# jorr3/Alphazero-4-player-chess

Hardware: AMD Instinct MI355X
Metric: MCTS simulations/sec (whole node), 256 games×400 sims, 10-block ResNet (higher is better)
Workload: dtype fp16

## Files before the change

### alphazero-4-player-chess_amd/csrc/fpc_tower.h

```cpp
#pragma once
#include <hip/hip_runtime.h>

#include <type_traits>

#include "fpc_tree_kernels.h"

namespace fpc {

typedef __attribute__((ext_vector_type(8))) __bf16 t_bf16x8;
typedef __attribute__((ext_vector_type(8))) _Float16 t_f16x8;
typedef __attribute__((ext_vector_type(4))) float t_f32x4;
typedef __attribute__((ext_vector_type(2))) float t_f32x2;
typedef __attribute__((ext_vector_type(4))) uint32_t t_u32x4;
typedef __attribute__((ext_vector_type(2))) uint32_t t_u32x2;
typedef __attribute__((ext_vector_type(2))) short t_i16x2;

template <int DT>
struct M16;
template <>
struct M16<0> {
  static __device__ __forceinline__ t_f32x4 mfma(t_u32x4 a, t_u32x4 b, t_f32x4 c) {
    return __builtin_amdgcn_mfma_f32_16x16x32_bf16(__builtin_bit_cast(t_bf16x8, a), __builtin_bit_cast(t_bf16x8, b), c, 0, 0, 0);
  }
  static __device__ __forceinline__ uint32_t pack2(float lo, float hi) {
    typedef __attribute__((ext_vector_type(2))) __bf16 b2;
    return __builtin_bit_cast(uint32_t, __builtin_convertvector((t_f32x2{lo, hi}), b2));
  }
  static __device__ __forceinline__ float lo(uint32_t p) { return __builtin_bit_cast(float, p << 16); }
  static __device__ __forceinline__ float hi(uint32_t p) { return __builtin_bit_cast(float, p & 0xffff0000u); }
};
template <>
struct M16<1> {
  static __device__ __forceinline__ t_f32x4 mfma(t_u32x4 a, t_u32x4 b, t_f32x4 c) {
    return __builtin_amdgcn_mfma_f32_16x16x32_f16(__builtin_bit_cast(t_f16x8, a), __builtin_bit_cast(t_f16x8, b), c, 0, 0, 0);
  }
  static __device__ __forceinline__ uint32_t pack2(float lo, float hi) {
    typedef __attribute__((ext_vector_type(2))) _Float16 h2;
    return __builtin_bit_cast(uint32_t, __builtin_convertvector((t_f32x2{lo, hi}), h2));
  }
  static __device__ __forceinline__ float lo(uint32_t p) { return (float)__builtin_bit_cast(_Float16, (uint16_t)(p & 0xffffu)); }
  static __device__ __forceinline__ float hi(uint32_t p) { return (float)__builtin_bit_cast(_Float16, (uint16_t)(p >> 16)); }
};
__device__ __forceinline__ uint32_t tw_relu2(uint32_t p) {
  return __builtin_bit_cast(uint32_t, __builtin_elementwise_max(__builtin_bit_cast(t_i16x2, p), (t_i16x2{0, 0})));
}

__host__ __device__ constexpr int tw_lay(int CH, int row, int c) {
  return (row >> 3) * (CH * 128) + (c >> 1) * 256 + (c & 1) * 128 + (row & 7) * 16;
}

constexpr int TW_THREADS = 256;
constexpr int TW_BIAS = 0;
constexpr int TW_DUMMY = 2048;
constexpr int TW_VRED = 2560;
constexpr int TW_BOARD = 2624;
constexpr int TW_PACE = 2944;
constexpr int TW_IMG0 = 4096;
constexpr int TW_IMG = 61440;
constexpr int TW_TAP = 32768;
constexpr int TW_RING = TW_IMG0 + TW_IMG;
constexpr int TW_LDS = TW_RING + 3 * TW_TAP;
constexpr int TW_STEM_TAP = 8192;
constexpr int TW_ENC = TW_RING + 9 * TW_STEM_TAP;
static_assert(TW_LDS == 163840, "k_tower uses the whole LDS of a CU");

struct TowerArgs {
  const fpc_board *boards;
  const int *leaf_slot, *leaf_turn;
  int board_stride;
  uint16_t one16;
  const uint16_t *in16;
  const unsigned char *Wstem;
  const float *bstem;
  const unsigned char *Wt;
  const float *bt;
  uint16_t *xfc;
  const float *vw;
  float *value;
  float vb;
  int L, P, R, PP, NR, T0, n_games, Kp, A_ch;
  int rules;
  unsigned long long *stamps;
};

__device__ __forceinline__ void tw_dma_8k(const unsigned char *gsrc_uniform, uint32_t lane_off, uint32_t lds_addr_uniform) {
  uint32_t keep;
  asm volatile(
      "s_mov_b32 %0, m0\n\ts_mov_b32 m0, %3\n\ts_nop 0\n\t"
      "global_load_lds_dwordx4 %1, %2\n\ts_add_u32 m0, m0, 0x400\n\tv_add_u32 %1, 0x400, %1\n\t"
      "global_load_lds_dwordx4 %1, %2\n\ts_add_u32 m0, m0, 0x400\n\tv_add_u32 %1, 0x400, %1\n\t"
      "global_load_lds_dwordx4 %1, %2\n\ts_add_u32 m0, m0, 0x400\n\tv_add_u32 %1, 0x400, %1\n\t"
      "global_load_lds_dwordx4 %1, %2\n\ts_add_u32 m0, m0, 0x400\n\tv_add_u32 %1, 0x400, %1\n\t"
      "global_load_lds_dwordx4 %1, %2\n\ts_add_u32 m0, m0, 0x400\n\tv_add_u32 %1, 0x400, %1\n\t"
      "global_load_lds_dwordx4 %1, %2\n\ts_add_u32 m0, m0, 0x400\n\tv_add_u32 %1, 0x400, %1\n\t"
      "global_load_lds_dwordx4 %1, %2\n\ts_add_u32 m0, m0, 0x400\n\tv_add_u32 %1, 0x400, %1\n\t"
      "global_load_lds_dwordx4 %1, %2\n\t"
      "s_mov_b32 m0, %0"
      : "=&s"(keep), "+v"(lane_off) : "s"(gsrc_uniform), "s"(lds_addr_uniform) : "memory", "scc");
}
__device__ __forceinline__ void tw_dma_4k(const unsigned char *gsrc_uniform, uint32_t lane_off, uint32_t lds_addr_uniform) {
  uint32_t keep;
  asm volatile(
      "s_mov_b32 %0, m0\n\ts_mov_b32 m0, %3\n\ts_nop 0\n\t"
      "global_load_lds_dwordx4 %1, %2\n\ts_add_u32 m0, m0, 0x400\n\tv_add_u32 %1, 0x400, %1\n\t"
      "global_load_lds_dwordx4 %1, %2\n\ts_add_u32 m0, m0, 0x400\n\tv_add_u32 %1, 0x400, %1\n\t"
      "global_load_lds_dwordx4 %1, %2\n\ts_add_u32 m0, m0, 0x400\n\tv_add_u32 %1, 0x400, %1\n\t"
      "global_load_lds_dwordx4 %1, %2\n\t"
      "s_mov_b32 m0, %0"
      : "=&s"(keep), "+v"(lane_off) : "s"(gsrc_uniform), "s"(lds_addr_uniform) : "memory", "scc");
}
template <int OFF>
__device__ __forceinline__ void tw_dma_piece(const unsigned char *gsrc_uniform, uint32_t lane_off) {
  asm volatile("global_load_lds_dwordx4 %0, %1 offset:%2" : : "v"(lane_off), "s"(gsrc_uniform), "i"(OFF) : "memory");
}
__device__ __forceinline__ void tw_set_m0(uint32_t lds_addr_uniform) {
  asm volatile("s_mov_b32 m0, %0\n\ts_nop 0" : : "s"(lds_addr_uniform) : "memory");
}
__device__ __forceinline__ void tw_dma_256(const unsigned char *gsrc_uniform, uint32_t lane_off, uint32_t lds_addr_uniform) {
  uint32_t keep;
  asm volatile("s_mov_b32 %0, m0\n\ts_mov_b32 m0, %3\n\ts_nop 0\n\tglobal_load_lds_dword %1, %2\n\ts_mov_b32 m0, %0"
               : "=&s"(keep) : "v"(lane_off), "s"(gsrc_uniform), "s"(lds_addr_uniform) : "memory");
}

#ifdef TW_STAMPS
#define TW_STAMP(GT, I)                                                                                       \
  do {                                                                                                        \
    if (g.stamps && blockIdx.x == 0 && ((GT) == TW_STAMPS || (GT) == TW_STAMPS + 1)) {                        \
      const unsigned long long t_ = __builtin_amdgcn_s_memtime();                                             \
      if (lane == 0) g.stamps[(((GT) - TW_STAMPS) * 8 + wave) * 16 + (I)] = t_;                               \
    }                                                                                                         \
  } while (0)
#else
#define TW_STAMP(GT, I) do {} while (0)
#endif
#ifndef TW_AHEAD
#define TW_AHEAD 2
#endif
#ifndef TW_LOADERS
#define TW_LOADERS 1
#endif
#ifndef TW_STAGGER
#define TW_STAGGER 3
#endif
#ifndef TW_STRIP
#define TW_STRIP 0
#endif
#ifndef TWC_LOADER_TILES
#define TWC_LOADER_TILES 6
#endif

#ifndef TWC_STAGGER
#define TWC_STAGGER 2
#endif

template <int DT, int MT, bool FAST, int NW, int LOAD, bool CMP = false, bool TU = false>
__device__ __forceinline__ void tw_body(const TowerArgs &g) {
  static_assert(!CMP || (!FAST && NW == 8 && TW_LOADERS == 1 && MT == (LOAD == 2 ? TWC_LOADER_TILES : 13 - TWC_LOADER_TILES)), "compact form: 8 waves, 13 row tiles");
  static_assert(!TU || (CMP && TW_STAGGER != 0 && TWC_STAGGER >= 1 && TWC_STAGGER <= 3), "tap-specialised loop: compact form with the burst stream");
  constexpr int CR = 14, CZ = 16;
  constexpr int TB0 = LOAD == 2 ? 0 : TWC_LOADER_TILES;
  constexpr int NT = NW * 64;
  constexpr int WN = NW / 2;
  constexpr int CT = 8 / WN;
  constexpr int PIECES = 4 * LOAD;
  constexpr int DMA_PER_WAVE = PIECES * 1024;
  constexpr int MID = PIECES == 8 ? 4096 : 0;
  constexpr bool STREAM = TW_AHEAD == 2 && !(TW_STAGGER != 0 && NW == 8 && TW_LOADERS == 1);
  constexpr int STAG = (NW == 8 && TW_LOADERS == 1 && LOAD == 0) ? (TU ? TWC_STAGGER : TW_STAGGER) : 0;
  extern __shared__ __attribute__((aligned(16))) unsigned char smem[];
  unsigned char *const img = smem + TW_IMG0;
  unsigned char *const ring = smem + TW_RING;
  const float *const biasbuf = reinterpret_cast<const float *>(smem + TW_BIAS);
  float *const vred = reinterpret_cast<float *>(smem + TW_VRED);
  fpc_board *const lboard = reinterpret_cast<fpc_board *>(smem + TW_BOARD);
  const int tid = threadIdx.x, lane = tid & 63;
  const int wave = __builtin_amdgcn_readfirstlane(tid >> 6);
  const int wm = wave / WN, wn = wave % WN;
  const int li = lane & 15, lq = lane >> 4;
  const int game = blockIdx.x;
  const int P = g.P, NR = g.NR;

  int slot = 0, rot_k = 0;
  if (g.boards) {
    slot = g.leaf_slot[game];
    if (slot < 0) return;
    rot_k = first_leaf_turn(g.leaf_slot, g.leaf_turn, g.n_games);
  }

  const int rbase = CMP ? CZ + TB0 * 16 + li : (g.T0 + wm * MT) * 16 + li;
  uint32_t inmask = 0;
#pragma unroll
  for (int mt = 0; mt < MT; ++mt) {
    const int r = rbase + 16 * mt;
    if (CMP) {
      if (r - CZ < CR * CR) inmask |= 1u << mt;
    } else {
      const int pi = r / P, pj = r - pi * P;
      if (r < g.PP && pi >= 1 && pi <= g.R && pj >= 1 && pj <= g.R) inmask |= 1u << mt;
    }
  }
  auto colmask = [](int mt, int dx) -> uint64_t {
    uint32_t m16 = 0;
    for (int i = 0; i < 16; ++i)
      if (dx != 0 && ((TB0 + mt) * 16 + i) % CR == (dx < 0 ? 0 : CR - 1)) m16 |= 1u << i;
    const uint32_t m32 = m16 * 0x10001u;
    return ((uint64_t)m32 << 32) | m32;
  };
  auto lane_select = [](uint32_t a, uint32_t b, uint64_t m) -> uint32_t {
    uint32_t r;
    asm("v_cndmask_b32_e64 %0, %1, %2, %3" : "=v"(r) : "v"(a), "v"(b), "s"(m));
    return r;
  };
  const int bq = (lq >> 1) * 256 + (lq & 1) * 128;
  const int apart = (li >> 3) * 2048 + (li & 7) * 16 + bq;
  const int apart_s = (li >> 3) * 512 + (li & 7) * 16 + bq;
  const int cb64 = wn * (CT * 16);
  const int cb16 = (wn & 1) * 16;
  const bool vactive = wn < 2;

  for (int c = tid; c < (TW_IMG0 + TW_IMG) / 16; c += NT) reinterpret_cast<t_u32x4 *>(smem)[c] = t_u32x4{0u, 0u, 0u, 0u};
  unsigned char *const enc = smem + TW_ENC;
  const int enc_bytes = CMP ? 240 * 64 : ((NR + 7) >> 3) * 512;
  for (int c = tid; c < enc_bytes / 16; c += NT) reinterpret_cast<t_u32x4 *>(enc)[c] = t_u32x4{0u, 0u, 0u, 0u};
  {
    const t_u32x4 *src = reinterpret_cast<const t_u32x4 *>(g.Wstem);
    t_u32x4 *dst = reinterpret_cast<t_u32x4 *>(ring);
    for (int c = tid; c < 9 * TW_STEM_TAP / 16; c += NT) dst[c] = src[c];
  }
  t_f32x4 bst[CT];
#pragma unroll
  for (int ct = 0; ct < CT; ++ct) bst[ct] = *reinterpret_cast<const t_f32x4 *>(g.bstem + cb64 + ct * 16 + 4 * lq);
  __syncthreads();
  if (g.boards) {
    constexpr int WPB = (int)(sizeof(fpc_board) / 4);
    if (tid < WPB) reinterpret_cast<uint32_t *>(lboard)[tid] =
        reinterpret_cast<const uint32_t *>(g.boards + (size_t)game * g.board_stride + slot)[tid];
    __syncthreads();
    if (g.rules & FPC_RULES_ROTATION) rot_k = lboard->turn;
    for (int r = tid; r < (CMP ? CR * CR : g.PP); r += NT) {
      const int pi = CMP ? r / CR + 1 : r / P, pj = CMP ? r % CR + 1 : r - pi * P;
      if (pi < 1 || pi > g.R || pj < 1 || pj > g.R) continue;
      const uint8_t p = lboard->sq[rot90_src(g.R, rot_k, pi - 1, pj - 1)];
      if (!present(p)) continue;
      const int plane = piece_plane(p, lboard->turn, g.rules);
      *reinterpret_cast<uint16_t *>(enc + tw_lay(4, CMP ? CZ + r : r, plane >> 3) + (plane & 7) * 2) = g.one16;
    }
  } else if (CMP) {
    const uint16_t *src = g.in16 + (size_t)game * g.PP * 32;
    for (int c = tid; c < CR * CR * 4; c += NT) {
      const int q = c >> 2, j = c & 3;
      *reinterpret_cast<t_u32x4 *>(enc + tw_lay(4, CZ + q, j)) =
          *reinterpret_cast<const t_u32x4 *>(src + ((size_t)(q / CR + 1) * P + q % CR + 1) * 32 + j * 8);
    }
  } else {
    const uint16_t *src = g.in16 + (size_t)game * g.PP * 32;
    for (int c = tid; c < NR * 4; c += NT) {
      const int r = c >> 2, j = c & 3;
      *reinterpret_cast<t_u32x4 *>(enc + tw_lay(4, r, j)) = *reinterpret_cast<const t_u32x4 *>(src + (size_t)r * 32 + j * 8);
    }
  }
  __syncthreads();

  t_f32x4 acc[MT][CT];
  t_u32x2 res[MT][CT];

  auto brow = [&](int mt, int shift) -> int {
    int r = rbase + 16 * mt + shift;
    r = r < 0 ? r + NR : r;
    r = r >= NR ? r - NR : r;
    return r;
  };

#pragma unroll
  for (int tap = 0; tap < 9; ++tap) {
    const int shift = (tap / 3 - 1) * (CMP ? CR : P) + (tap % 3 - 1);
    t_u32x4 fa[CT], fb[MT];
#pragma unroll
    for (int ct = 0; ct < CT; ++ct)
      fa[ct] = *reinterpret_cast<const t_u32x4 *>(ring + tap * TW_STEM_TAP + (cb64 + ct * 16) * 64 + apart_s);
#pragma unroll
    for (int mt = 0; mt < MT; ++mt) {
      const int r = CMP ? (int)lane_select((uint32_t)(rbase + 16 * mt + shift), (uint32_t)((rbase + shift) & 7), colmask(mt, tap % 3 - 1)) : brow(mt, shift);
      fb[mt] = *reinterpret_cast<const t_u32x4 *>(enc + (r >> 3) * 512 + (r & 7) * 16 + bq);
    }
#pragma unroll
    for (int mt = 0; mt < MT; ++mt)
#pragma unroll
      for (int ct = 0; ct < CT; ++ct) acc[mt][ct] = M16<DT>::mfma(fa[ct], fb[mt], tap == 0 ? bst[ct] : acc[mt][ct]);
  }
  __syncthreads();

  const int total = (g.L + 2) * 9;
  const uint32_t dma_lane = (uint32_t)lane * 16u;
  const int lw = LOAD == 2 ? (wave & 3) : wave;
  auto issue_bias = [&](int T) {
    if (T % 9 == 0 && T < total && wave < 4) {
      const int l = T / 9;
      tw_dma_256(reinterpret_cast<const unsigned char *>(g.bt + (size_t)l * 256 + wave * 64), (uint32_t)lane * 4u,
                 (uint32_t)__builtin_amdgcn_readfirstlane(TW_BIAS + ((l & 1) * 256 + wave * 64) * 4));
    }
  };
  auto issue_tap = [&](int T) {
    issue_bias(T);
    if (LOAD == 0 || (TW_STRIP & 4)) return;
    const unsigned char *src = g.Wt + (size_t)T * TW_TAP + lw * DMA_PER_WAVE;
    const uint32_t dst = (uint32_t)__builtin_amdgcn_readfirstlane(TW_RING + (T % 3) * TW_TAP + lw * DMA_PER_WAVE);
    if (PIECES == 8) tw_dma_8k(src, dma_lane, dst);
    else tw_dma_4k(src, dma_lane, dst);
  };
  const unsigned char *dsrc = g.Wt;
  auto open_tap = [&](int T) {
    issue_bias(T);
    if (LOAD == 0) return;
    dsrc = g.Wt + (size_t)T * TW_TAP + lw * DMA_PER_WAVE + MID;
    tw_set_m0((uint32_t)__builtin_amdgcn_readfirstlane(TW_RING + (T % 3) * TW_TAP + lw * DMA_PER_WAVE + MID));
  };
  auto piece = [&](auto i_c) {
    constexpr int I = decltype(i_c)::value;
    if (LOAD != 0) tw_dma_piece<I * 1024 - MID>(dsrc, dma_lane);
  };
  issue_tap(0);
  issue_tap(1);
  if (STREAM) {
    open_tap(2);
    piece(std::integral_constant<int, 0>{});
    if (LOAD == 2) piece(std::integral_constant<int, 1>{});
  }

  unsigned char *const dummy = smem + TW_DUMMY + lane * 8;
  unsigned char *const wbase = img + (rbase >> 3) * 2048 + (rbase & 7) * 16 + wn * (CT * 256) + (lane >> 5) * 128 + ((lane >> 4) & 1) * 8;
  auto epilogue = [&](auto res_c) {
    constexpr int RES = decltype(res_c)::value;
    if (TW_STRIP & 16) return;
#pragma unroll
    for (int mt = 0; mt < MT; ++mt) {
      unsigned char *dst = ((inmask >> mt) & 1u) ? wbase + mt * 4096 : dummy;
#pragma unroll
      for (int ct = 0; ct < CT; ++ct) {
        t_f32x4 v = acc[mt][ct];
        if (RES == 2) {
          v[0] += M16<DT>::lo(res[mt][ct][0]); v[1] += M16<DT>::hi(res[mt][ct][0]);
          v[2] += M16<DT>::lo(res[mt][ct][1]); v[3] += M16<DT>::hi(res[mt][ct][1]);
        }
        const t_u32x2 pk = t_u32x2{tw_relu2(M16<DT>::pack2(v[0], v[1])), tw_relu2(M16<DT>::pack2(v[2], v[3]))};
        if (RES != 0) res[mt][ct] = pk;
        *reinterpret_cast<t_u32x2 *>(((inmask >> mt) & 1u) ? dst + ct * 256 : dst) = pk;
      }
      __builtin_amdgcn_sched_barrier(0);
    }
  };
  const std::integral_constant<int, 0> c0{};
  const std::integral_constant<int, 1> c1{};
  const std::integral_constant<int, 2> c2{};
  const std::integral_constant<int, 3> c3{};
  epilogue(c1);
  if (TW_STRIP & 32) { asm volatile("s_waitcnt vmcnt(0)" ::: "memory"); return; }
  if (STREAM) asm volatile("s_waitcnt vmcnt(%0)" ::"n"(PIECES + LOAD) : "memory");
  else asm volatile("s_waitcnt vmcnt(0)" ::: "memory");
  __syncthreads();

  t_u32x4 fa[2][CT], fb[2][MT];
  int gt = 0;
  const unsigned char *wslot;
  const unsigned char *bbase;
  const unsigned char *blast;
  int boff[FAST ? 1 : MT];
  auto set_tap = [&](int tap, int cb) {
    wslot = ring + (gt % 3) * TW_TAP + cb * 256 + apart;
    const int shift = (tap / 3 - 1) * P + (tap % 3 - 1);
    if (FAST) {
      const int r = rbase + shift;
      bbase = img + (r >> 3) * 2048 + (r & 7) * 16 + bq;
      int rl = r + 16 * (MT - 1);
      rl = rl >= NR ? rl - NR : rl;
      blast = img + (rl >> 3) * 2048 + (rl & 7) * 16 + bq;
    } else if (CMP) {
      const int dx = tap % 3 - 1;
      const int r = rbase + (tap / 3 - 1) * CR + dx;
      const uint32_t zoff = (r & 7) * 16 + bq;
      const uint32_t b0 = (r >> 3) * 2048 + zoff;
#pragma unroll
      for (int mt = 0; mt < MT; ++mt) {
        const uint64_t m = dx < 0 ? colmask(mt, -1) : dx > 0 ? colmask(mt, 1) : 0ull;
        boff[mt] = (int)lane_select(b0 + mt * 4096, zoff, m);
      }
    } else {
#pragma unroll
      for (int mt = 0; mt < MT; ++mt) {
        const int r = brow(mt, shift);
        boff[mt] = (r >> 3) * 2048 + (r & 7) * 16 + bq;
      }
    }
  };
  const unsigned char *wrow = nullptr, *wrow2 = nullptr;
  auto set_wrow = [&](int cb) {
    int o = cb * 256 + apart, o2 = o + 2 * TW_TAP;
    asm volatile("" : "+v"(o2));
    wrow = ring + o;
    wrow2 = ring + o2;
  };
  int rrow = rbase - CR;
  auto set_tap_u = [&](auto xn_c) {
    constexpr int XN = decltype(xn_c)::value;
    wslot = XN == 2 ? wrow2 : wrow + XN * TW_TAP;
    const int r = rrow + (XN - 1);
    const uint32_t zoff = (r & 7) * 16 + bq;
    const uint32_t b0 = (r >> 3) * 2048 + zoff;
#pragma unroll
    for (int mt = 0; mt < MT; ++mt)
      boff[mt] = XN == 1 ? (int)(b0 + mt * 4096) : (int)lane_select(b0 + mt * 4096, zoff, colmask(mt, XN - 1));
  };
  auto bptr = [&](int mt) -> const unsigned char * {
    if (FAST) return mt == MT - 1 ? blast : bbase + mt * 4096;
    return img + boff[mt];
  };
  auto kstep = [&](auto mode_c, auto buf_c, auto ksn_c, auto bias_c, const t_f32x4 *b4, auto q_c) {
    constexpr int MODE = decltype(mode_c)::value, B = decltype(buf_c)::value, KSN = decltype(ksn_c)::value;
    constexpr bool BIAS = decltype(bias_c)::value != 0;
    constexpr int N = B ^ 1, Q = decltype(q_c)::value;
    if (!(TW_STRIP & 2)) {
#pragma unroll
      for (int ct = 0; ct < CT; ++ct) fa[N][ct] = *reinterpret_cast<const t_u32x4 *>(wslot + ct * 4096 + KSN * 512);
      fb[N][0] = *reinterpret_cast<const t_u32x4 *>(bptr(0) + KSN * 512);
    }
    __builtin_amdgcn_sched_barrier(0);
#pragma unroll
    for (int mt = 0; mt < MT; ++mt) {
      if (TW_STRIP & 1) {
        if (BIAS) {
#pragma unroll
          for (int ct = 0; ct < (MODE == 0 ? CT : 1); ++ct) acc[mt][ct] = b4[ct];
        }
        asm volatile("" : "+v"(fa[B][0]), "+v"(fb[B][mt]));
      } else if (MODE == 0) {
#pragma unroll
        for (int ct = 0; ct < CT; ++ct) acc[mt][ct] = M16<DT>::mfma(fa[B][ct], fb[B][mt], BIAS ? b4[ct] : acc[mt][ct]);
      } else if (NW == 4 || vactive) {
        acc[mt][0] = M16<DT>::mfma(fa[B][0], fb[B][mt], BIAS ? b4[0] : acc[mt][0]);
      }
      __builtin_amdgcn_sched_barrier(0);
      if (mt + 1 < MT && !(TW_STRIP & 2)) {
        fb[N][mt + 1] = *reinterpret_cast<const t_u32x4 *>(bptr(mt + 1) + KSN * 512);
        __builtin_amdgcn_sched_barrier(0);
      }
      if (STREAM && LOAD != 0) {
        if (mt == (LOAD == 2 ? MT / 3 : MT / 2)) piece(std::integral_constant<int, LOAD * Q>{});
        if (LOAD == 2 && mt == (2 * MT) / 3) piece(std::integral_constant<int, LOAD * Q + 1>{});
        __builtin_amdgcn_sched_barrier(0);
      }
    }
  };
  auto load_b0 = [&]() {
#pragma unroll
    for (int mt = 0; mt < MT; ++mt) fb[0][mt] = *reinterpret_cast<const t_u32x4 *>(bptr(mt));
  };
  const unsigned char *usrc = g.Wt + (size_t)TW_TAP + lw * DMA_PER_WAVE;
  const uint32_t udst = (uint32_t)__builtin_amdgcn_readfirstlane(TW_RING + lw * DMA_PER_WAVE);
  auto tap_u = [&](auto mode_c, auto x_c, const t_f32x4 *b4, const int dy, const int cb_next) {
    constexpr int X = decltype(x_c)::value;
    if (STAG == 2) {
      TW_STAMP(gt, 3);
      __syncthreads();
      TW_STAMP(gt, 4);
    }
    TW_STAMP(gt, 0);
    kstep(mode_c, c1, c2, c0, b4, c2);
    TW_STAMP(gt, 1);
    if (STAG == 1) __syncthreads();
    kstep(mode_c, c0, c3, c0, b4, c3);
    TW_STAMP(gt, 2);
    if (!STAG) {
      asm volatile("s_waitcnt vmcnt(0)" ::: "memory");
      TW_STAMP(gt, 3);
      if (!(TW_STRIP & 8)) __syncthreads();
      TW_STAMP(gt, 4);
      if (LOAD != 0 && !(TW_STRIP & 4)) {
        usrc += TW_TAP;
        tw_dma_8k(usrc, dma_lane, udst + ((X + 2) % 3) * TW_TAP);
      }
      TW_STAMP(gt, 5);
    }
    ++gt;
    if (X == 2) {
      rrow = dy == 1 ? rbase - CR : rrow + CR;
      if (dy == 1) set_wrow(cb_next);
    }
    set_tap_u(std::integral_constant<int, (X + 1) % 3>{});
    TW_STAMP(gt - 1, 6);
    kstep(mode_c, c1, c0, c0, b4, c0);
    TW_STAMP(gt - 1, 7);
  };
  auto run_layer = [&](auto mode_c, const int layer, const int cb, const int cb_next) {
    constexpr int MODE = decltype(mode_c)::value;
    if (TU && wave < 4 && layer + 1 < g.L + 2)
      tw_dma_256(reinterpret_cast<const unsigned char *>(g.bt + (size_t)(layer + 1) * 256 + wave * 64), (uint32_t)lane * 4u,
                 (uint32_t)__builtin_amdgcn_readfirstlane(TW_BIAS + (((layer + 1) & 1) * 256 + wave * 64) * 4));
    t_f32x4 b4[CT];
    {
      const float *bl = biasbuf + (layer & 1) * 256 + cb + 4 * lq;
#pragma unroll
      for (int ct = 0; ct < (MODE == 0 ? CT : 1); ++ct) b4[ct] = *reinterpret_cast<const t_f32x4 *>(bl + ct * 16);
    }
    if (STAG == 3 && !(TW_STRIP & 8)) __syncthreads();
    kstep(mode_c, c0, c1, c1, b4, c1);
    if (TU) {
#pragma unroll 1
      for (int dy = -1;; ++dy) {
        tap_u(mode_c, c0, b4, dy, cb_next);
        if (STAG == 3 && !(TW_STRIP & 8)) __syncthreads();
        kstep(mode_c, c0, c1, c0, b4, c1);
        TW_STAMP(gt - 1, 8);
        tap_u(mode_c, c1, b4, dy, cb_next);
        if (STAG == 3 && !(TW_STRIP & 8)) __syncthreads();
        kstep(mode_c, c0, c1, c0, b4, c1);
        TW_STAMP(gt - 1, 8);
        tap_u(mode_c, c2, b4, dy, cb_next);
        if (dy == 1) break;
        if (STAG == 3 && !(TW_STRIP & 8)) __syncthreads();
        kstep(mode_c, c0, c1, c0, b4, c1);
        TW_STAMP(gt - 1, 8);
      }
      TW_STAMP(gt - 1, 8);
      return;
    }
#pragma unroll 1
    for (int tap = 0; tap < 9; ++tap) {
      if (STAG == 2) {
        TW_STAMP(gt, 3);
        __syncthreads();
        TW_STAMP(gt, 4);
      }
      TW_STAMP(gt, 0);
      kstep(mode_c, c1, c2, c0, b4, c2);
      TW_STAMP(gt, 1);
      if (STAG == 1) __syncthreads();
      kstep(mode_c, c0, c3, c0, b4, c3);
      TW_STAMP(gt, 2);
      if (!STAG) {
        if (STREAM) asm volatile("s_waitcnt vmcnt(%0)" ::"n"(PIECES) : "memory");
        else asm volatile("s_waitcnt vmcnt(0)" ::: "memory");
        TW_STAMP(gt, 3);
        if (!(TW_STRIP & 8)) __syncthreads();
        TW_STAMP(gt, 4);
        if (STREAM) open_tap(gt + 3);
        else if (gt + 2 < total) issue_tap(gt + 2);
        TW_STAMP(gt, 5);
      }
      ++gt;
      set_tap(tap == 8 ? 0 : tap + 1, tap == 8 ? cb_next : cb);
      TW_STAMP(gt - 1, 6);
      kstep(mode_c, c1, c0, c0, b4, c0);
      TW_STAMP(gt - 1, 7);
      if (STAG == 3 && tap < 8 && !(TW_STRIP & 8)) __syncthreads();
      if (tap < 8) kstep(mode_c, c0, c1, c0, b4, c1);
      TW_STAMP(gt - 1, 8);
    }
  };

  if (TU) {
    set_wrow(cb64);
    set_tap_u(c0);
  } else {
    set_tap(0, cb64);
  }
#pragma unroll
  for (int ct = 0; ct < CT; ++ct) fa[0][ct] = *reinterpret_cast<const t_u32x4 *>(wslot + ct * 4096);
  load_b0();
  const int nblocks = g.L / 2;
#pragma unroll 1
  for (int blk = 0; blk < nblocks; ++blk) {
    run_layer(c0, 2 * blk, cb64, cb64);
    epilogue(c0);
    __syncthreads();
    load_b0();
    run_layer(c0, 2 * blk + 1, cb64, blk + 1 == nblocks ? cb16 : cb64);
    epilogue(c2);
    __syncthreads();
    load_b0();
  }
  float vpart = 0.f;
  {
    run_layer(c1, g.L, cb16, cb64);
#pragma unroll
    for (int mt = 0; mt < MT; ++mt) {
      const int r = rbase + 16 * mt;
      const int pi = r / P, pj = r - pi * P;
      const bool in = ((inmask >> mt) & 1u) && (NW == 4 || vactive);
      const int qp = !in ? 0 : CMP ? r - CZ : (pi - 1) * g.R + (pj - 1);
      const t_f32x4 w4 = *reinterpret_cast<const t_f32x4 *>(g.vw + qp * 32 + cb16 + 4 * lq);
#pragma unroll
      for (int j = 0; j < 4; ++j) {
        float v = acc[mt][0][j];
        v = v > 0.f ? v : 0.f;
        vpart += in ? v * w4[j] : 0.f;
      }
    }
  }
  run_layer(c0, g.L + 1, cb64, cb64);
  epilogue(c0);
  __syncthreads();

  if (!(TW_STRIP & 64)) {
    const int cpr = g.A_ch / 8;
    for (int c = tid; c < (CMP ? CR * CR : g.PP) * 16; c += NT) {
      const int j = c & 15;
      if (j >= cpr) continue;
      int r = c >> 4, q = r;
      if (CMP) r += CZ;
      else {
        const int pi = r / P, pj = r - pi * P;
        if (pi < 1 || pi > g.R || pj < 1 || pj > g.R) continue;
        q = (pi - 1) * g.R + (pj - 1);
      }
      *reinterpret_cast<t_u32x4 *>(g.xfc + (size_t)game * g.Kp + (size_t)q * g.A_ch + j * 8) =
          *reinterpret_cast<const t_u32x4 *>(img + tw_lay(16, r, j));
    }
  }
  for (int off = 32; off >= 1; off >>= 1) vpart += __shfl_xor(vpart, off);
  if (lane == 0) vred[wave] = vpart;
  __syncthreads();
  if (tid == 0) g.value[game] = tanhf(g.vb + ((vred[0] + vred[1]) + (vred[WN] + vred[WN + 1])));
  asm volatile("s_waitcnt vmcnt(0)" ::: "memory");
}

template <int DT, int MT, bool FAST, int NW>
__global__ void __launch_bounds__(NW * 64, NW / 4) k_tower(TowerArgs g) {
  if (NW == 8 && TW_LOADERS == 1) {
    if (__builtin_amdgcn_readfirstlane(threadIdx.x >> 6) < 4) tw_body<DT, MT, FAST, NW, 2>(g);
    else tw_body<DT, MT, FAST, NW, 0>(g);
  } else {
    tw_body<DT, MT, FAST, NW, NW == 4 ? 2 : 1>(g);
  }
}

template <int DT, bool TU>
__global__ void __launch_bounds__(512, 2) k_towerc(TowerArgs g) {
  if (__builtin_amdgcn_readfirstlane(threadIdx.x >> 6) < 4) tw_body<DT, TWC_LOADER_TILES, false, 8, 2, true, TU>(g);
  else tw_body<DT, 13 - TWC_LOADER_TILES, false, 8, 0, true, TU>(g);
}

__global__ void __launch_bounds__(256) k_tower_prep(const uint16_t *W, unsigned char *out, int taps, int cin) {
  const int CH = cin / 8;
  const long c = (long)blockIdx.x * 256 + threadIdx.x;
  if (c >= (long)taps * 128 * CH) return;
  const int tap = (int)(c / (128 * CH)), rem = (int)(c % (128 * CH)), row = rem / CH, j = rem % CH;
  *reinterpret_cast<t_u32x4 *>(out + (size_t)tap * 128 * cin * 2 + tw_lay(CH, row, j)) =
      *reinterpret_cast<const t_u32x4 *>(W + ((size_t)tap * 128 + row) * cin + j * 8);
}

}
```

Baseline: 496,700.

## Overlap tower prologue: register stem weights, early tap DMA, single-wave board load

Restructures the tower kernel prologue. The stem filter is loaded straight into registers instead of copied into the LDS ring, and the first two trunk weight taps are DMA'd before the stem conv runs. The leaf board and rotation are fetched by one wave into LDS, and the compact input is prefetched into registers. The kernel also skips some redundant weight DMA issues for later layer modes. The aim is to hide global-memory latency and drop barriers at kernel start, at the cost of more register pressure and more intricate ordering logic.

```diff
diff --git a/alphazero-4-player-chess_amd/csrc/fpc_tower.h b/alphazero-4-player-chess_amd/csrc/fpc_tower.h
--- a/alphazero-4-player-chess_amd/csrc/fpc_tower.h
+++ b/alphazero-4-player-chess_amd/csrc/fpc_tower.h
@@ -54,6 +54,7 @@
 constexpr int TW_DUMMY = 2048;
 constexpr int TW_VRED = 2560;
 constexpr int TW_BOARD = 2624;
+constexpr int TW_ROT = 2912;
 constexpr int TW_PACE = 2944;
 constexpr int TW_IMG0 = 4096;
 constexpr int TW_IMG = 61440;
@@ -154,7 +155,7 @@
 #endif
 
 template <int DT, int MT, bool FAST, int NW, int LOAD, bool CMP = false, bool TU = false>
-__device__ __forceinline__ void tw_body(const TowerArgs &g) {
+__device__ __forceinline__ void tw_body(const TowerArgs &g, const int slot) {
   static_assert(!CMP || (!FAST && NW == 8 && TW_LOADERS == 1 && MT == (LOAD == 2 ? TWC_LOADER_TILES : 13 - TWC_LOADER_TILES)), "compact form: 8 waves, 13 row tiles");
   static_assert(!TU || (CMP && TW_STAGGER != 0 && TWC_STAGGER >= 1 && TWC_STAGGER <= 3), "tap-specialised loop: compact form with the burst stream");
   constexpr int CR = 14, CZ = 16;
@@ -180,115 +181,33 @@
   const int game = blockIdx.x;
   const int P = g.P, NR = g.NR;
 
-  int slot = 0, rot_k = 0;
-  if (g.boards) {
-    slot = g.leaf_slot[game];
-    if (slot < 0) return;
-    rot_k = first_leaf_turn(g.leaf_slot, g.leaf_turn, g.n_games);
-  }
-
-  const int rbase = CMP ? CZ + TB0 * 16 + li : (g.T0 + wm * MT) * 16 + li;
-  uint32_t inmask = 0;
-#pragma unroll
-  for (int mt = 0; mt < MT; ++mt) {
-    const int r = rbase + 16 * mt;
-    if (CMP) {
-      if (r - CZ < CR * CR) inmask |= 1u << mt;
-    } else {
-      const int pi = r / P, pj = r - pi * P;
-      if (r < g.PP && pi >= 1 && pi <= g.R && pj >= 1 && pj <= g.R) inmask |= 1u << mt;
-    }
-  }
-  auto colmask = [](int mt, int dx) -> uint64_t {
-    uint32_t m16 = 0;
-    for (int i = 0; i < 16; ++i)
-      if (dx != 0 && ((TB0 + mt) * 16 + i) % CR == (dx < 0 ? 0 : CR - 1)) m16 |= 1u << i;
-    const uint32_t m32 = m16 * 0x10001u;
-    return ((uint64_t)m32 << 32) | m32;
-  };
-  auto lane_select = [](uint32_t a, uint32_t b, uint64_t m) -> uint32_t {
-    uint32_t r;
-    asm("v_cndmask_b32_e64 %0, %1, %2, %3" : "=v"(r) : "v"(a), "v"(b), "s"(m));
-    return r;
-  };
+  const int cb64 = wn * (CT * 16);
   const int bq = (lq >> 1) * 256 + (lq & 1) * 128;
-  const int apart = (li >> 3) * 2048 + (li & 7) * 16 + bq;
   const int apart_s = (li >> 3) * 512 + (li & 7) * 16 + bq;
-  const int cb64 = wn * (CT * 16);
-  const int cb16 = (wn & 1) * 16;
-  const bool vactive = wn < 2;
-
-  for (int c = tid; c < (TW_IMG0 + TW_IMG) / 16; c += NT) reinterpret_cast<t_u32x4 *>(smem)[c] = t_u32x4{0u, 0u, 0u, 0u};
-  unsigned char *const enc = smem + TW_ENC;
-  const int enc_bytes = CMP ? 240 * 64 : ((NR + 7) >> 3) * 512;
-  for (int c = tid; c < enc_bytes / 16; c += NT) reinterpret_cast<t_u32x4 *>(enc)[c] = t_u32x4{0u, 0u, 0u, 0u};
-  {
-    const t_u32x4 *src = reinterpret_cast<const t_u32x4 *>(g.Wstem);
-    t_u32x4 *dst = reinterpret_cast<t_u32x4 *>(ring);
-    for (int c = tid; c < 9 * TW_STEM_TAP / 16; c += NT) dst[c] = src[c];
-  }
+  constexpr int SG = CT == 2 ? 9 : 3;
+  t_u32x4 fs[SG][CT];
+  auto load_fs = [&](int tap0) {
+#pragma unroll
+    for (int t = 0; t < SG; ++t)
+#pragma unroll
+      for (int ct = 0; ct < CT; ++ct)
+        fs[t][ct] = *reinterpret_cast<const t_u32x4 *>(g.Wstem + (tap0 + t) * TW_STEM_TAP + (cb64 + ct * 16) * 64 + apart_s);
+  };
+  load_fs(0);
   t_f32x4 bst[CT];
 #pragma unroll
   for (int ct = 0; ct < CT; ++ct) bst[ct] = *reinterpret_cast<const t_f32x4 *>(g.bstem + cb64 + ct * 16 + 4 * lq);
-  __syncthreads();
-  if (g.boards) {
-    constexpr int WPB = (int)(sizeof(fpc_board) / 4);
-    if (tid < WPB) reinterpret_cast<uint32_t *>(lboard)[tid] =
-        reinterpret_cast<const uint32_t *>(g.boards + (size_t)game * g.board_stride + slot)[tid];
-    __syncthreads();
-    if (g.rules & FPC_RULES_ROTATION) rot_k = lboard->turn;
-    for (int r = tid; r < (CMP ? CR * CR : g.PP); r += NT) {
-      const int pi = CMP ? r / CR + 1 : r / P, pj = CMP ? r % CR + 1 : r - pi * P;
-      if (pi < 1 || pi > g.R || pj < 1 || pj > g.R) continue;
-      const uint8_t p = lboard->sq[rot90_src(g.R, rot_k, pi - 1, pj - 1)];
-      if (!present(p)) continue;
-      const int plane = piece_plane(p, lboard->turn, g.rules);
-      *reinterpret_cast<uint16_t *>(enc + tw_lay(4, CMP ? CZ + r : r, plane >> 3) + (plane & 7) * 2) = g.one16;
-    }
-  } else if (CMP) {
+  constexpr int XCH = CMP ? (CR * CR * 4 + NT - 1) / NT : 1;
+  t_u32x4 xin[XCH];
+  if (CMP && !g.boards) {
     const uint16_t *src = g.in16 + (size_t)game * g.PP * 32;
-    for (int c = tid; c < CR * CR * 4; c += NT) {
-      const int q = c >> 2, j = c & 3;
-      *reinterpret_cast<t_u32x4 *>(enc + tw_lay(4, CZ + q, j)) =
-          *reinterpret_cast<const t_u32x4 *>(src + ((size_t)(q / CR + 1) * P + q % CR + 1) * 32 + j * 8);
-    }
-  } else {
-    const uint16_t *src = g.in16 + (size_t)game * g.PP * 32;
-    for (int c = tid; c < NR * 4; c += NT) {
-      const int r = c >> 2, j = c & 3;
-      *reinterpret_cast<t_u32x4 *>(enc + tw_lay(4, r, j)) = *reinterpret_cast<const t_u32x4 *>(src + (size_t)r * 32 + j * 8);
-    }
-  }
-  __syncthreads();
-
-  t_f32x4 acc[MT][CT];
-  t_u32x2 res[MT][CT];
-
-  auto brow = [&](int mt, int shift) -> int {
-    int r = rbase + 16 * mt + shift;
-    r = r < 0 ? r + NR : r;
-    r = r >= NR ? r - NR : r;
-    return r;
-  };
-
-#pragma unroll
-  for (int tap = 0; tap < 9; ++tap) {
-    const int shift = (tap / 3 - 1) * (CMP ? CR : P) + (tap % 3 - 1);
-    t_u32x4 fa[CT], fb[MT];
-#pragma unroll
-    for (int ct = 0; ct < CT; ++ct)
-      fa[ct] = *reinterpret_cast<const t_u32x4 *>(ring + tap * TW_STEM_TAP + (cb64 + ct * 16) * 64 + apart_s);
-#pragma unroll
-    for (int mt = 0; mt < MT; ++mt) {
-      const int r = CMP ? (int)lane_select((uint32_t)(rbase + 16 * mt + shift), (uint32_t)((rbase + shift) & 7), colmask(mt, tap % 3 - 1)) : brow(mt, shift);
-      fb[mt] = *reinterpret_cast<const t_u32x4 *>(enc + (r >> 3) * 512 + (r & 7) * 16 + bq);
-    }
-#pragma unroll
-    for (int mt = 0; mt < MT; ++mt)
-#pragma unroll
-      for (int ct = 0; ct < CT; ++ct) acc[mt][ct] = M16<DT>::mfma(fa[ct], fb[mt], tap == 0 ? bst[ct] : acc[mt][ct]);
-  }
-  __syncthreads();
+#pragma unroll
+    for (int i = 0; i < XCH; ++i) {
+      const int c = tid + i * NT, q = c < CR * CR * 4 ? c >> 2 : 0, j = c & 3;
+      xin[i] = *reinterpret_cast<const t_u32x4 *>(src + ((size_t)(q / CR + 1) * P + q % CR + 1) * 32 + j * 8);
+    }
+  }
+  if (slot < 0) { asm volatile("s_waitcnt vmcnt(0)" ::: "memory"); return; }
 
   const int total = (g.L + 2) * 9;
   const uint32_t dma_lane = (uint32_t)lane * 16u;
@@ -308,6 +227,105 @@
     if (PIECES == 8) tw_dma_8k(src, dma_lane, dst);
     else tw_dma_4k(src, dma_lane, dst);
   };
+  issue_tap(0);
+  issue_tap(1);
+
+  if (g.boards && (NW == 4 || LOAD == 0) && wave == NW - 1) {
+    constexpr int WPB = (int)(sizeof(fpc_board) / 4);
+    static_assert(WPB <= 128 && TW_BOARD + WPB * 4 <= TW_ROT, "the leaf board: two words per lane, in front of TW_ROT");
+    const uint32_t *bsrc = reinterpret_cast<const uint32_t *>(g.boards + (size_t)game * g.board_stride + slot);
+    const uint32_t w0 = bsrc[lane < WPB ? lane : 0], w1 = bsrc[lane + 64 < WPB ? lane + 64 : lane];
+    const int rot = first_leaf_turn(g.leaf_slot, g.leaf_turn, g.n_games);
+    if (lane < WPB) reinterpret_cast<uint32_t *>(lboard)[lane] = w0;
+    if (lane + 64 < WPB) reinterpret_cast<uint32_t *>(lboard)[lane + 64] = w1;
+    if (lane == 0) *reinterpret_cast<int *>(smem + TW_ROT) = rot;
+  }
+
+  const int rbase = CMP ? CZ + TB0 * 16 + li : (g.T0 + wm * MT) * 16 + li;
+  uint32_t inmask = 0;
+#pragma unroll
+  for (int mt = 0; mt < MT; ++mt) {
+    const int r = rbase + 16 * mt;
+    if (CMP) {
+      if (r - CZ < CR * CR) inmask |= 1u << mt;
+    } else {
+      const int pi = r / P, pj = r - pi * P;
+      if (r < g.PP && pi >= 1 && pi <= g.R && pj >= 1 && pj <= g.R) inmask |= 1u << mt;
+    }
+  }
+  auto colmask = [](int mt, int dx) -> uint64_t {
+    uint32_t m16 = 0;
+    for (int i = 0; i < 16; ++i)
+      if (dx != 0 && ((TB0 + mt) * 16 + i) % CR == (dx < 0 ? 0 : CR - 1)) m16 |= 1u << i;
+    const uint32_t m32 = m16 * 0x10001u;
+    return ((uint64_t)m32 << 32) | m32;
+  };
+  auto lane_select = [](uint32_t a, uint32_t b, uint64_t m) -> uint32_t {
+    uint32_t r;
+    asm("v_cndmask_b32_e64 %0, %1, %2, %3" : "=v"(r) : "v"(a), "v"(b), "s"(m));
+    return r;
+  };
+  const int apart = (li >> 3) * 2048 + (li & 7) * 16 + bq;
+  const int cb16 = (wn & 1) * 16;
+  const bool vactive = wn < 2;
+
+  for (int c = tid + TW_IMG0 / 16; c < (TW_IMG0 + TW_IMG) / 16; c += NT) reinterpret_cast<t_u32x4 *>(smem)[c] = t_u32x4{0u, 0u, 0u, 0u};
+  unsigned char *const enc = smem + TW_ENC;
+  const int enc_bytes = CMP ? 240 * 64 : ((NR + 7) >> 3) * 512;
+  for (int c = tid; c < enc_bytes / 16; c += NT) reinterpret_cast<t_u32x4 *>(enc)[c] = t_u32x4{0u, 0u, 0u, 0u};
+  __syncthreads();
+  if (g.boards) {
+    const int rot_k = (g.rules & FPC_RULES_ROTATION) ? (int)lboard->turn : *reinterpret_cast<const int *>(smem + TW_ROT);
+    for (int r = tid; r < (CMP ? CR * CR : g.PP); r += NT) {
+      const int pi = CMP ? r / CR + 1 : r / P, pj = CMP ? r % CR + 1 : r - pi * P;
+      if (pi < 1 || pi > g.R || pj < 1 || pj > g.R) continue;
+      const uint8_t p = lboard->sq[rot90_src(g.R, rot_k, pi - 1, pj - 1)];
+      if (!present(p)) continue;
+      const int plane = piece_plane(p, lboard->turn, g.rules);
+      *reinterpret_cast<uint16_t *>(enc + tw_lay(4, CMP ? CZ + r : r, plane >> 3) + (plane & 7) * 2) = g.one16;
+    }
+  } else if (CMP) {
+#pragma unroll
+    for (int i = 0; i < XCH; ++i) {
+      const int c = tid + i * NT;
+      if (c < CR * CR * 4) *reinterpret_cast<t_u32x4 *>(enc + tw_lay(4, CZ + (c >> 2), c & 3)) = xin[i];
+    }
+  } else {
+    const uint16_t *src = g.in16 + (size_t)game * g.PP * 32;
+    for (int c = tid; c < NR * 4; c += NT) {
+      const int r = c >> 2, j = c & 3;
+      *reinterpret_cast<t_u32x4 *>(enc + tw_lay(4, r, j)) = *reinterpret_cast<const t_u32x4 *>(src + (size_t)r * 32 + j * 8);
+    }
+  }
+  __syncthreads();
+
+  t_f32x4 acc[MT][CT];
+  t_u32x2 res[MT][CT];
+
+  auto brow = [&](int mt, int shift) -> int {
+    int r = rbase + 16 * mt + shift;
+    r = r < 0 ? r + NR : r;
+    r = r >= NR ? r - NR : r;
+    return r;
+  };
+
+#pragma unroll
+  for (int tap = 0; tap < 9; ++tap) {
+    const int shift = (tap / 3 - 1) * (CMP ? CR : P) + (tap % 3 - 1);
+    t_u32x4 fb[MT];
+    if (SG < 9 && tap != 0 && tap % SG == 0) load_fs(tap);
+#pragma unroll
+    for (int mt = 0; mt < MT; ++mt) {
+      const int r = CMP ? (int)lane_select((uint32_t)(rbase + 16 * mt + shift), (uint32_t)((rbase + shift) & 7), colmask(mt, tap % 3 - 1)) : brow(mt, shift);
+      fb[mt] = *reinterpret_cast<const t_u32x4 *>(enc + (r >> 3) * 512 + (r & 7) * 16 + bq);
+    }
+#pragma unroll
+    for (int mt = 0; mt < MT; ++mt)
+#pragma unroll
+      for (int ct = 0; ct < CT; ++ct) acc[mt][ct] = M16<DT>::mfma(fs[tap % SG][ct], fb[mt], tap == 0 ? bst[ct] : acc[mt][ct]);
+  }
+  if (STREAM) __syncthreads();
+
   const unsigned char *dsrc = g.Wt;
   auto open_tap = [&](int T) {
     issue_bias(T);
@@ -319,8 +337,6 @@
     constexpr int I = decltype(i_c)::value;
     if (LOAD != 0) tw_dma_piece<I * 1024 - MID>(dsrc, dma_lane);
   };
-  issue_tap(0);
-  issue_tap(1);
   if (STREAM) {
     open_tap(2);
     piece(std::integral_constant<int, 0>{});
@@ -476,7 +492,7 @@
       TW_STAMP(gt, 4);
       if (LOAD != 0 && !(TW_STRIP & 4)) {
         usrc += TW_TAP;
-        tw_dma_8k(usrc, dma_lane, udst + ((X + 2) % 3) * TW_TAP);
+        if (decltype(mode_c)::value == 0 || lw == 0 || (X != 0 && dy == 1)) tw_dma_8k(usrc, dma_lane, udst + ((X + 2) % 3) * TW_TAP);
       }
       TW_STAMP(gt, 5);
     }
@@ -543,7 +559,7 @@
         if (!(TW_STRIP & 8)) __syncthreads();
         TW_STAMP(gt, 4);
         if (STREAM) open_tap(gt + 3);
-        else if (gt + 2 < total) issue_tap(gt + 2);
+        else if (gt + 2 < total && (MODE == 0 || lw * DMA_PER_WAVE < 8192 || tap >= 7)) issue_tap(gt + 2);
         TW_STAMP(gt, 5);
       }
       ++gt;
@@ -625,18 +641,20 @@
 
 template <int DT, int MT, bool FAST, int NW>
 __global__ void __launch_bounds__(NW * 64, NW / 4) k_tower(TowerArgs g) {
+  const int slot = g.boards ? g.leaf_slot[blockIdx.x] : 0;
   if (NW == 8 && TW_LOADERS == 1) {
-    if (__builtin_amdgcn_readfirstlane(threadIdx.x >> 6) < 4) tw_body<DT, MT, FAST, NW, 2>(g);
-    else tw_body<DT, MT, FAST, NW, 0>(g);
+    if (__builtin_amdgcn_readfirstlane(threadIdx.x >> 6) < 4) tw_body<DT, MT, FAST, NW, 2>(g, slot);
+    else tw_body<DT, MT, FAST, NW, 0>(g, slot);
   } else {
-    tw_body<DT, MT, FAST, NW, NW == 4 ? 2 : 1>(g);
+    tw_body<DT, MT, FAST, NW, NW == 4 ? 2 : 1>(g, slot);
   }
 }
 
 template <int DT, bool TU>
 __global__ void __launch_bounds__(512, 2) k_towerc(TowerArgs g) {
-  if (__builtin_amdgcn_readfirstlane(threadIdx.x >> 6) < 4) tw_body<DT, TWC_LOADER_TILES, false, 8, 2, true, TU>(g);
-  else tw_body<DT, 13 - TWC_LOADER_TILES, false, 8, 0, true, TU>(g);
+  const int slot = g.boards ? g.leaf_slot[blockIdx.x] : 0;
+  if (__builtin_amdgcn_readfirstlane(threadIdx.x >> 6) < 4) tw_body<DT, TWC_LOADER_TILES, false, 8, 2, true, TU>(g, slot);
+  else tw_body<DT, 13 - TWC_LOADER_TILES, false, 8, 0, true, TU>(g, slot);
 }
 
 __global__ void __launch_bounds__(256) k_tower_prep(const uint16_t *W, unsigned char *out, int taps, int cin) {
```

Result: no change. 498,200 (median of 3 runs) (+0.3%).
